# satoutahhaithem/gym

Measured on AMD Instinct MI355X. Metric: strategy-step param GB/s (%HBM/xGMI peak) + ms/outer step, GPT-2 124M, 1-8 GPUs, higher is better.
Workload: dtype f32

## Files before the change

### gym_amd/csrc/demo_wave.hip

```cpp
#include "ga_common.h"

namespace ga {
namespace dw {

constexpr int kWaves = 8;
constexpr int kThreads = 64 * kWaves;
constexpr int kLd = 65;
constexpr int kCand = 128;
static_assert(2 * (kCand + 64) >= 320, "the fallback top-k keeps its maps in lst[128..319]");

typedef float f32x16 __attribute__((ext_vector_type(16)));

#ifdef GA_DEMO_STAMPS
extern __device__ unsigned long long* g_demo_stamps_w;
#define DW_PH_DECL unsigned long long ph_acc[16] = {}, ph_last = __builtin_amdgcn_s_memtime()
#define DW_PH(i)                                                    \
    do {                                                            \
        const unsigned long long t_ = __builtin_amdgcn_s_memtime(); \
        ph_acc[i] += t_ - ph_last;                                  \
        ph_last = t_;                                               \
    } while (0)
#define DW_CNT(i) (ph_acc[i] += 1)
#define DW_PH_FLUSH()                                                                                       \
    do {                                                                                                    \
        if ((threadIdx.x & 63) == 0) {                                                                      \
            unsigned long long* row_ = g_demo_stamps_w + ((size_t)blockIdx.x * kWaves + (threadIdx.x >> 6)) * 16; \
            for (int i_ = 0; i_ < 16; ++i_) row_[i_] = ph_acc[i_];                                          \
        }                                                                                                   \
    } while (0)
#else
#define DW_PH_DECL do {} while (0)
#define DW_PH(i) do {} while (0)
#define DW_CNT(i) do {} while (0)
#define DW_PH_FLUSH() do {} while (0)
#endif

#define WAVE_LDS_SYNC() asm volatile("" ::: "memory")

__device__ __forceinline__ int lane_id() {
    int t = (int)threadIdx.x;
    asm volatile("" : "+v"(t));
    return t & 63;
}

__device__ __forceinline__ f32x16 zero16() {
    f32x16 a;
#pragma unroll
    for (int r = 0; r < 16; ++r) a[r] = 0.f;
    return a;
}

__device__ __forceinline__ f32x16 mfma(float a, float b, const f32x16& c) {
    return __builtin_amdgcn_mfma_f32_32x32x2f32(a, b, c, 0, 0, 0);
}

__device__ __forceinline__ constexpr int rowmap(int r, int h) { return (r & 3) + 8 * (r >> 2) + 4 * h; }

__device__ __forceinline__ int blk(int h, int q) { return h ? 4 + q : (q < 4 ? q : 8 + q); }

__device__ __forceinline__ int pi_col(int H, int m) { return 4 * blk((m >> 2) & 1, 4 * H + (m >> 3)) + (m & 3); }

__device__ __forceinline__ float basis64(const float* Hb, int i, int d) {
    const float v = Hb[(i < 32 ? i : 63 - i) * kLd + d];
    return (i >= 32 && (d & 1)) ? -v : v;
}

__device__ __forceinline__ uint32_t keyv(float v) { return (__float_as_uint(v) & 0x7fffffffu) + 1u; }

__device__ __forceinline__ int wave_excl_scan128(int v) {
    int r = 0;
#pragma unroll
    for (int b = 0; b < 7; ++b) {
        const uint64_t m = __ballot((v >> b) & 1);
        r += (int)__builtin_amdgcn_mbcnt_hi((uint32_t)(m >> 32), __builtin_amdgcn_mbcnt_lo((uint32_t)m, 0u)) << b;
    }
    return r;
}

__device__ __forceinline__ int wave_sum(int v) {
#pragma unroll
    for (int d = 32; d > 0; d >>= 1) v += __shfl_xor(v, d, 64);
    return v;
}

__device__ __forceinline__ int find_tensor(const ga_demo_tensor* __restrict__ T, int ntens, int tix, int chunk) {
    int lo = tix < 0 ? 0 : tix, hi = ntens - 1;
    while (lo < hi) {
        const int mid = (lo + hi + 1) >> 1;
        if (T[mid].chunk_start <= chunk) lo = mid;
        else hi = mid - 1;
    }
    return lo;
}

__device__ __forceinline__ void decode_wave_priority() {
    const int w = __builtin_amdgcn_readfirstlane((int)threadIdx.x >> 6);
    asm volatile("s_cmp_lt_u32 %0, 4\n\ts_cbranch_scc1 1f\n\ts_setprio 1\n1:" ::"s"(w) : "scc");
}

__device__ __forceinline__ uint32_t rdl(uint32_t v, int j) {
    return (uint32_t)__builtin_amdgcn_readlane((int)v, j);
}

struct ListLDS {
    uint32_t lst[2 * (kCand + 64)];
    uint32_t bm[128];
    uint32_t sm[4];
};

struct WaveLDS : ListLDS {
    float tile[64 * kLd];
};

__device__ __forceinline__ uint32_t lane_off(int s, int q, int l, int h, int stride) {
    return (uint32_t)((s ? 63 - l : l) * stride + 4 * blk(h, q));
}

template <typename T>
__device__ __forceinline__ const T* at_off(const T* pb, uint32_t off) {
    return reinterpret_cast<const T*>(reinterpret_cast<const char*>(pb) + (uint64_t)(uint32_t)(off * (uint32_t)sizeof(T)));
}
template <typename T>
__device__ __forceinline__ T* at_off(T* pb, uint32_t off) {
    return reinterpret_cast<T*>(reinterpret_cast<char*>(pb) + (uint64_t)(uint32_t)(off * (uint32_t)sizeof(T)));
}

template <typename T>
__device__ __forceinline__ void load_rows(const T* pb, int stride, int l, int h, bool vec, int nrows,
                                          float (&o)[2][8][4]) {
    if (vec && nrows == 64) {
#pragma unroll
        for (int s = 0; s < 2; ++s)
#pragma unroll
            for (int q = 0; q < 8; ++q)
                Vec4<T>::unpack(*reinterpret_cast<const typename Vec4<T>::type*>(at_off(pb, lane_off(s, q, l, h, stride))),
                                o[s][q]);
        return;
    }
#pragma unroll
    for (int s = 0; s < 2; ++s) {
        const bool live = (s ? 63 - l : l) < nrows;
#pragma unroll
        for (int q = 0; q < 8; ++q) {
            const T* a = at_off(pb, lane_off(s, q, l, h, stride));
            if (live && vec) {
                Vec4<T>::unpack(*reinterpret_cast<const typename Vec4<T>::type*>(a), o[s][q]);
            } else {
#pragma unroll
                for (int e = 0; e < 4; ++e) o[s][q][e] = live ? Elem<T>::load(a + e) : 0.f;
            }
        }
    }
}

template <typename T>
__device__ __forceinline__ void store_rows(T* pb, int stride, int l, int h, bool vec, int nrows,
                                           const float (&o)[2][8][4]) {
    if (vec && nrows == 64) {
#pragma unroll
        for (int s = 0; s < 2; ++s)
#pragma unroll
            for (int q = 0; q < 8; ++q)
                *reinterpret_cast<typename Vec4<T>::type*>(at_off(pb, lane_off(s, q, l, h, stride))) = Vec4<T>::pack(o[s][q]);
        return;
    }
#pragma unroll
    for (int s = 0; s < 2; ++s) {
        if ((s ? 63 - l : l) >= nrows) continue;
#pragma unroll
        for (int q = 0; q < 8; ++q) {
            T* a = at_off(pb, lane_off(s, q, l, h, stride));
            if (vec) {
                *reinterpret_cast<typename Vec4<T>::type*>(a) = Vec4<T>::pack(o[s][q]);
            } else {
#pragma unroll
                for (int e = 0; e < 4; ++e) Elem<T>::store(a + e, o[s][q][e]);
            }
        }
    }
}

template <typename T>
__device__ __forceinline__ void error_feedback(T* param, const T* grad, const T* delta, int stride, int l, int h,
                                               bool vec, int nrows, float lr, float decay, float wd_factor,
                                               float (&x)[2][8][4]) {
    if (wd_factor != 1.f) {
        load_rows(param, stride, l, h, vec, nrows, x);
#pragma unroll
        for (int s = 0; s < 2; ++s)
#pragma unroll
            for (int q = 0; q < 8; ++q)
#pragma unroll
                for (int e = 0; e < 4; ++e) x[s][q][e] *= wd_factor;
        store_rows(param, stride, l, h, vec, nrows, x);
    }
    float g[2][8][4];
    load_rows(delta, stride, l, h, vec, nrows, x);
    load_rows(grad, stride, l, h, vec, nrows, g);
#pragma unroll
    for (int s = 0; s < 2; ++s)
#pragma unroll
        for (int q = 0; q < 8; ++q)
#pragma unroll
            for (int e = 0; e < 4; ++e)
                x[s][q][e] = fmaf(lr, g[s][q][e], decay != 1.f ? x[s][q][e] * decay : x[s][q][e]);
}

__device__ __forceinline__ void row_product_half(const float (&xs)[8][4], const float* Hb, int l, int h,
                                                 f32x16 (&Ts)[2]) {
#pragma unroll
    for (int qc = 0; qc < 2; ++qc) {
        f32x16 acc = zero16();
#pragma unroll
        for (int t = 0; t < 16; ++t) {
            const int q = t >> 2, e = t & 3;
            const float u = xs[q][e], w = xs[7 - q][3 - e];
            const float a = qc ? u - w : u + w;
            acc = mfma(a, Hb[(16 * h + t) * kLd + 2 * l + qc], acc);
        }
        Ts[qc] = acc;
    }
}

__device__ __forceinline__ void row_product(const float (&x)[2][8][4], const float* Hb, int l, int h,
                                            f32x16 (&T)[2][2]) {
#pragma unroll
    for (int s = 0; s < 2; ++s) {
#pragma unroll
        for (int qc = 0; qc < 2; ++qc) {
            f32x16 acc = zero16();
#pragma unroll
            for (int t = 0; t < 16; ++t) {
                const int q = t >> 2, e = t & 3;
                const float u = x[s][q][e], w = x[s][7 - q][3 - e];
                const float a = qc ? u - w : u + w;
                acc = mfma(a, Hb[(16 * h + t) * kLd + 2 * l + qc], acc);
            }
            T[s][qc] = acc;
        }
    }
}

constexpr int kSynB = 4;

__device__ __forceinline__ void parity_lists(uint32_t epos, uint32_t ebits, bool ent, int lane, uint2* lstp,
                                             int& np0, int& np1) {
    const int pl = (int)((epos >> 6) & 1u);
    const uint64_t m0 = __ballot(ent && pl == 0), m1 = __ballot(ent && pl == 1);
    const uint64_t mm = pl ? m1 : m0;
    const int ix = (int)__builtin_amdgcn_mbcnt_hi((uint32_t)(mm >> 32), __builtin_amdgcn_mbcnt_lo((uint32_t)mm, 0u));
    const int E0 = __popcll(m0), E1 = __popcll(m1);
    const int P0 = (E0 + 1) & ~1, P1 = (E1 + 1) & ~1;
    WAVE_LDS_SYNC();
    if (ent) lstp[pl * 64 + ix] = make_uint2(epos, ebits);
    if (lane == 0 && E0 < P0) lstp[E0] = make_uint2(0u, 0u);
    if (lane == 1 && E1 < P1) lstp[64 + E1] = make_uint2(0u, 0u);
    WAVE_LDS_SYNC();
    np0 = P0 >> 1;
    np1 = P1 >> 1;
}

template <int B>
__device__ __forceinline__ void synth_batch(const uint2* lst, int q, int cH, int l, int h, const float* Hb,
                                            f32x16& acc) {
    uint2 e[B];
#pragma unroll
    for (int u = 0; u < B; ++u) e[u] = lst[2 * (q + u) + h];
    float a[B], b[B];
#pragma unroll
    for (int u = 0; u < B; ++u) {
        const int bq = (int)(e[u].x >> 6), dq = (int)(e[u].x & 63);
        a[u] = __uint_as_float(e[u].y) * basis64(Hb, cH, dq);
        b[u] = Hb[l * kLd + bq];
    }
#pragma unroll
    for (int u = 0; u < B; ++u) acc = mfma(a[u], b[u], acc);
}

__device__ __forceinline__ void synth_list(const uint2* lst, int np, int cH, int l, int h, const float* Hb,
                                           f32x16& acc) {
    static_assert(kSynB == 2 || kSynB == 4 || kSynB == 8, "synthesis tail handles 4/2/1 pairs");
    int q = 0;
    for (; q + kSynB <= np; q += kSynB) synth_batch<kSynB>(lst, q, cH, l, h, Hb, acc);
    const int rem = np - q;
    if (kSynB > 4 && (rem & 4)) {
        synth_batch<4>(lst, q, cH, l, h, Hb, acc);
        q += 4;
    }
    if (kSynB > 2 && (rem & 2)) {
        synth_batch<2>(lst, q, cH, l, h, Hb, acc);
        q += 2;
    }
    if (rem & 1) synth_batch<1>(lst, q, cH, l, h, Hb, acc);
}

__device__ __forceinline__ void synth_half(const uint2* lstp, int np0, int np1, int H, int l, int h,
                                           const float* Hb, f32x16& Re, f32x16& Ro) {
    const int cH = pi_col(H, l);
    Re = zero16();
    Ro = zero16();
    synth_list(lstp, np0, cH, l, h, Hb, Re);
    synth_list(lstp + 64, np1, cH, l, h, Hb, Ro);
}

__device__ __forceinline__ uint32_t coal_off(int i, int lane, int stride) {
    return (uint32_t)(((lane >> 4) + 4 * i) * stride + 4 * (lane & 15));
}

template <typename T, int I0 = 0, int NI = 16>
__device__ __forceinline__ void load_coal(const T* pb, int stride, bool vec, int lane, float (&o)[16][4]) {
    if (vec) {
#pragma unroll
        for (int i = I0; i < I0 + NI; ++i)
            Vec4<T>::unpack(*reinterpret_cast<const typename Vec4<T>::type*>(at_off(pb, coal_off(i, lane, stride))),
                            o[i]);
    } else {
#pragma unroll
        for (int i = I0; i < I0 + NI; ++i)
#pragma unroll
            for (int e = 0; e < 4; ++e) o[i][e] = Elem<T>::load(at_off(pb, coal_off(i, lane, stride)) + e);
    }
}

template <typename T>
__device__ __forceinline__ void store_vec(T* pb, uint32_t off, const typename Vec4<T>::type& v) {
    *reinterpret_cast<typename Vec4<T>::type*>(at_off(pb, off)) = v;
}

template <typename T>
__device__ __forceinline__ void store_coal(T* pb, int stride, bool vec, int lane, const float (&o)[16][4]) {
    if (vec) {
#pragma unroll
        for (int i = 0; i < 16; ++i) store_vec(pb, coal_off(i, lane, stride), Vec4<T>::pack(o[i]));
    } else {
#pragma unroll
        for (int i = 0; i < 16; ++i)
#pragma unroll
            for (int e = 0; e < 4; ++e) Elem<T>::store(at_off(pb, coal_off(i, lane, stride)) + e, o[i][e]);
    }
}

__device__ __forceinline__ int t4(int row, int cb) { return row * 16 + (cb ^ (row & 15)); }


template <typename T>
__device__ __forceinline__ void chunk64_tail(const f32x16 (&Y)[2][2], int k, T* delta, int cols, bool vec,
                                             int32_t* out_idx, float* out_val, const float* Hb, ListLDS& W,
                                             float4* tile
#ifdef GA_DEMO_STAMPS
                                             , unsigned long long (&ph_acc)[16], unsigned long long& ph_last
#endif
) {
    const int lane = lane_id(), l = lane & 31, h = lane >> 5;
    __builtin_amdgcn_s_setprio(1);
    auto posof = [&](int par, int qc, int r) -> uint32_t {
        return (uint32_t)((2 * rowmap(r, h) + par) * 64 + 2 * l + qc);
    };
    float mymaxf = 0.f;
#pragma unroll
    for (int par = 0; par < 2; ++par)
#pragma unroll
        for (int qc = 0; qc < 2; ++qc)
#pragma unroll
            for (int r = 0; r < 16; ++r) mymaxf = fmaxf(mymaxf, fabsf(Y[par][qc][r]));
    const uint32_t mymax = keyv(mymaxf);
    uint32_t T0 = 0;
#pragma unroll
    for (int bit = 30; bit >= 19; --bit) {
        const uint32_t cnd = T0 | (1u << bit);
        if (__popcll(__ballot(mymax >= cnd)) >= k) T0 = cnd;
    }
    if (T0 == 0u) T0 = 1u;
    const float T0f = __uint_as_float(T0 - 1u);
    int mine = 0;
#pragma unroll
    for (int par = 0; par < 2; ++par)
#pragma unroll
        for (int qc = 0; qc < 2; ++qc)
#pragma unroll
            for (int r = 0; r < 16; ++r) mine += fabsf(Y[par][qc][r]) >= T0f ? 1 : 0;
    const int excl = wave_excl_scan128(mine);
    const int incl = excl + mine;
    const int C = __builtin_amdgcn_readlane(incl, 63);
    DW_PH(10);
    W.bm[2 * lane] = 0u;
    W.bm[2 * lane + 1] = 0u;
    if (C <= kCand) {
        uint2* L2 = reinterpret_cast<uint2*>(W.lst);
        float T0c = T0f;
        asm volatile("" : "+v"(T0c));
        int at = excl;
#pragma unroll
        for (int par = 0; par < 2; ++par)
#pragma unroll
            for (int qc = 0; qc < 2; ++qc)
#pragma unroll
                for (int r = 0; r < 16; ++r) {
                    const float v = Y[par][qc][r];
                    const bool cnd = fabsf(v) >= T0c;
                    L2[cnd ? at : kCand + lane] = make_uint2(posof(par, qc, r), __float_as_uint(v));
                    at += cnd ? 1 : 0;
                }
        WAVE_LDS_SYNC();
        DW_PH(11);
        uint32_t pos[2], bits[2], key[2];
        bool ok[2];
#pragma unroll
        for (int e = 0; e < 2; ++e) {
            const int g = e * 64 + lane;
            ok[e] = g < C;
            const uint2 pb = L2[ok[e] ? g : kCand + lane];
            pos[e] = ok[e] ? pb.x : 0u;
            bits[e] = pb.y;
            key[e] = ok[e] ? keyv(__uint_as_float(pb.y)) : 0u;
            if (ok[e]) atomicOr(&W.bm[pos[e] >> 5], 1u << (pos[e] & 31));
        }
        WAVE_LDS_SYNC();
        const uint32_t w0 = W.bm[2 * lane], w1 = W.bm[2 * lane + 1];
        const int cnt = __popc(w0) + __popc(w1);
        const int pre = wave_excl_scan128(cnt);
        int rank[2];
#pragma unroll
        for (int e = 0; e < 2; ++e) {
            const int Lw = (int)(pos[e] >> 6);
            const uint64_t pair = ((uint64_t)(uint32_t)__shfl((int)w1, Lw, 64) << 32) |
                                  (uint32_t)__shfl((int)w0, Lw, 64);
            const int preL = __shfl(pre, Lw, 64);
            rank[e] = ok[e] ? preL + __popcll(pair & ((1ull << (pos[e] & 63)) - 1ull)) : 0x7fff;
        }
        DW_PH(12);
        uint32_t thr = 0;
        for (int bit = 31; bit >= 0; --bit) {
            const uint32_t cnd = thr | (1u << bit);
            if (__popcll(__ballot(key[0] >= cnd)) + __popcll(__ballot(key[1] >= cnd)) >= k) thr = cnd;
        }
        const int need = k - __popcll(__ballot(key[0] > thr)) - __popcll(__ballot(key[1] > thr));
        const uint64_t q0 = __ballot(key[0] == thr), q1 = __ballot(key[1] == thr);
        bool sel[2];
        if (__popcll(q0) + __popcll(q1) == need) {
            sel[0] = key[0] >= thr;
            sel[1] = key[1] >= thr;
        } else {
            int tr[2] = {0, 0};
            for (uint64_t m = q0; m; m &= m - 1) {
                const int rj = __builtin_amdgcn_readlane(rank[0], __builtin_ctzll(m));
                tr[0] += rj < rank[0];
                tr[1] += rj < rank[1];
            }
            for (uint64_t m = q1; m; m &= m - 1) {
                const int rj = __builtin_amdgcn_readlane(rank[1], __builtin_ctzll(m));
                tr[0] += rj < rank[0];
                tr[1] += rj < rank[1];
            }
            sel[0] = key[0] > thr || (key[0] == thr && tr[0] < need);
            sel[1] = key[1] > thr || (key[1] == thr && tr[1] < need);
        }
        DW_PH(13);
        if (lane < 4) W.sm[lane] = 0u;
        WAVE_LDS_SYNC();
#pragma unroll
        for (int e = 0; e < 2; ++e)
            if (sel[e]) atomicOr(&W.sm[rank[e] >> 5], 1u << (rank[e] & 31));
        WAVE_LDS_SYNC();
        const uint64_t m0 = ((uint64_t)W.sm[1] << 32) | W.sm[0], m1 = ((uint64_t)W.sm[3] << 32) | W.sm[2];
#pragma unroll
        for (int e = 0; e < 2; ++e) {
            if (sel[e]) {
                const int r = rank[e];
                const int slot = r < 64 ? __popcll(m0 & ((1ull << r) - 1ull))
                                        : __popcll(m0) + __popcll(m1 & ((1ull << (r - 64)) - 1ull));
                W.lst[2 * slot] = pos[e];
                W.lst[2 * slot + 1] = bits[e];
                out_idx[slot] = (int32_t)pos[e];
                out_val[slot] = __uint_as_float(bits[e]);
            }
        }
        WAVE_LDS_SYNC();
    } else {
        DW_CNT(8);
        auto opq = [](float v) {
            asm volatile("" : "+v"(v));
            return v;
        };
        auto lane_pos = [&]() {
            uint32_t lp = (uint32_t)(512 * h + 2 * l);
            asm volatile("" : "+v"(lp));
            return lp;
        };
        auto pos_c = [](int par, int qc, int r) -> uint32_t {
            return (uint32_t)((2 * ((r & 3) + 8 * (r >> 2)) + par) * 64 + qc);
        };
        uint32_t thr = 0;
        for (int bit = 31; bit >= 0; --bit) {
            const uint32_t cnd = thr | (1u << bit);
            const float f = __uint_as_float(cnd - 1u);
            int cl = 0;
#pragma unroll
            for (int par = 0; par < 2; ++par)
#pragma unroll
                for (int qc = 0; qc < 2; ++qc)
#pragma unroll
                    for (int r = 0; r < 16; ++r) cl += fabsf(opq(Y[par][qc][r])) >= f ? 1 : 0;
            if (wave_sum(cl) >= k) thr = cnd;
        }
        int gl = 0;
        {
            const uint32_t lp = lane_pos();
#pragma unroll
            for (int par = 0; par < 2; ++par)
#pragma unroll
                for (int qc = 0; qc < 2; ++qc)
#pragma unroll
                    for (int r = 0; r < 16; ++r) {
                        const uint32_t kv = keyv(opq(Y[par][qc][r]));
                        gl += kv > thr ? 1 : 0;
                        if (kv == thr) {
                            const uint32_t p = lp + pos_c(par, qc, r);
                            atomicOr(&W.bm[p >> 5], 1u << (p & 31));
                        }
                    }
        }
        const int need = k - wave_sum(gl);
        WAVE_LDS_SYNC();
        uint32_t* preL = W.lst + 128;
        {
            const uint32_t w0 = W.bm[2 * lane], w1 = W.bm[2 * lane + 1];
            preL[lane] = (uint32_t)wave_excl_scan128(__popc(w0) + __popc(w1));
        }
        WAVE_LDS_SYNC();
        uint32_t* sel = W.lst + 192;
        sel[2 * lane] = 0u;
        sel[2 * lane + 1] = 0u;
        WAVE_LDS_SYNC();
        {
            const uint32_t lp = lane_pos();
#pragma unroll
            for (int par = 0; par < 2; ++par)
#pragma unroll
                for (int qc = 0; qc < 2; ++qc)
#pragma unroll
                    for (int r = 0; r < 16; ++r) {
                        const uint32_t kv = keyv(opq(Y[par][qc][r]));
                        const uint32_t p = lp + pos_c(par, qc, r);
                        bool s = kv > thr;
                        if (kv == thr) {
                            const uint32_t Lw = p >> 6;
                            const uint64_t pair = ((uint64_t)W.bm[2 * Lw + 1] << 32) | W.bm[2 * Lw];
                            const int tr = (int)preL[Lw] + __popcll(pair & ((1ull << (p & 63)) - 1ull));
                            s = tr < need;
                        }
                        if (s) atomicOr(&sel[p >> 5], 1u << (p & 31));
                    }
        }
        WAVE_LDS_SYNC();
        {
            const uint32_t w0 = sel[2 * lane], w1 = sel[2 * lane + 1];
            preL[lane] = (uint32_t)wave_excl_scan128(__popc(w0) + __popc(w1));
        }
        WAVE_LDS_SYNC();
        {
            const uint32_t lp = lane_pos();
#pragma unroll
            for (int par = 0; par < 2; ++par)
#pragma unroll
                for (int qc = 0; qc < 2; ++qc)
#pragma unroll
                    for (int r = 0; r < 16; ++r) {
                        const uint32_t p = lp + pos_c(par, qc, r);
                        const uint32_t Lw = p >> 6;
                        const uint64_t pair = ((uint64_t)sel[2 * Lw + 1] << 32) | sel[2 * Lw];
                        if ((pair >> (p & 63)) & 1ull) {
                            const int slot = (int)preL[Lw] + __popcll(pair & ((1ull << (p & 63)) - 1ull));
                            const float v = opq(Y[par][qc][r]);
                            W.lst[2 * slot] = p;
                            W.lst[2 * slot + 1] = __float_as_uint(v);
                            out_idx[slot] = (int32_t)p;
                            out_val[slot] = v;
                        }
                    }
        }
        WAVE_LDS_SYNC();
    }
    DW_PH(3);
    __builtin_amdgcn_s_setprio(0);
    uint2* lstp = reinterpret_cast<uint2*>(W.lst);
    int np0, np1;
    parity_lists(lane < k ? W.lst[2 * lane] : 0u, lane < k ? W.lst[2 * lane + 1] : 0u, lane < k, lane, lstp, np0,
                 np1);
#pragma unroll
    for (int H = 0; H < 2; ++H) {
        f32x16 Re, Ro;
        synth_half(lstp, np0, np1, H, l, h, Hb, Re, Ro);
#pragma unroll
        for (int qq = 0; qq < 4; ++qq)
#pragma unroll
            for (int s = 0; s < 2; ++s) {
                float4& v = tile[t4(s ? 63 - l : l, blk(h, 4 * H + qq))];
                float4 o = v;
                const int r = 4 * qq;
                o.x -= s ? Re[r] - Ro[r] : Re[r] + Ro[r];
                o.y -= s ? Re[r + 1] - Ro[r + 1] : Re[r + 1] + Ro[r + 1];
                o.z -= s ? Re[r + 2] - Ro[r + 2] : Re[r + 2] + Ro[r + 2];
                o.w -= s ? Re[r + 3] - Ro[r + 3] : Re[r + 3] + Ro[r + 3];
                v = o;
            }
        DW_PH(4);
    }
    WAVE_LDS_SYNC();
    {
        float o[16][4];
#pragma unroll
        for (int i = 0; i < 16; ++i) {
            const float4 v = tile[t4((lane >> 4) + 4 * i, lane & 15)];
            o[i][0] = v.x;
            o[i][1] = v.y;
            o[i][2] = v.z;
            o[i][3] = v.w;
        }
        store_coal(delta, cols, vec, lane, o);
    }
    WAVE_LDS_SYNC();
    DW_PH(5);
}

template <typename T>
__device__ __forceinline__ void chunk64(const ga_demo_tensor& td, int c, T* param, const T* grad, T* delta,
                                        int32_t* out_idx, float* out_val, float lr, float decay, float wd_factor,
                                        int ptr_vec, const float* Hb, WaveLDS& W
#ifdef GA_DEMO_STAMPS
                                        , unsigned long long (&ph_acc)[16], unsigned long long& ph_last
#endif
) {
    const int cy = c / td.gx, cx = c - cy * td.gx;
    const int64_t base = td.offset + (int64_t)cy * 64 * td.cols + (int64_t)cx * 64;
    param += base;
    grad += base;
    delta += base;
    const bool vec = ptr_vec && (td.offset % 4 == 0) && (td.cols % 4 == 0);
    float4* tile = reinterpret_cast<float4*>(W.tile);
    {
        const int lane = lane_id();
        if (wd_factor != 1.f) {
            float pv[16][4];
            load_coal(param, td.cols, vec, lane, pv);
#pragma unroll
            for (int i = 0; i < 16; ++i)
#pragma unroll
                for (int e = 0; e < 4; ++e) pv[i][e] *= wd_factor;
            store_coal(param, td.cols, vec, lane, pv);
        }
    }
    f32x16 Y[2][2];
    {
        const int lane = lane_id(), l = lane & 31, h = lane >> 5;
        float Dv[16][4], Gv[16][4];
        __builtin_amdgcn_s_setprio(2);
        load_coal<T, 0, 8>(delta, td.cols, vec, lane, Dv);
        load_coal<T, 0, 8>(grad, td.cols, vec, lane, Gv);
        __builtin_amdgcn_sched_barrier(0);
        load_coal<T, 8, 8>(delta, td.cols, vec, lane, Dv);
        load_coal<T, 8, 8>(grad, td.cols, vec, lane, Gv);
#pragma unroll
        for (int i = 0; i < 8; ++i)
            asm volatile("" : "+v"(Dv[i][0]), "+v"(Dv[i][1]), "+v"(Dv[i][2]), "+v"(Dv[i][3]), "+v"(Gv[i][0]),
                              "+v"(Gv[i][1]), "+v"(Gv[i][2]), "+v"(Gv[i][3])::"memory");
        __builtin_amdgcn_s_setprio(0);
        f32x16 Tm[2][2];
#pragma unroll
        for (int s = 0; s < 2; ++s) {
#pragma unroll
            for (int i = 8 * s; i < 8 * s + 8; ++i) {
                if (s == 1)
                    asm volatile("" : "+v"(Dv[i][0]), "+v"(Dv[i][1]), "+v"(Dv[i][2]), "+v"(Dv[i][3]),
                                      "+v"(Gv[i][0]), "+v"(Gv[i][1]), "+v"(Gv[i][2]), "+v"(Gv[i][3]));
                float v[4];
#pragma unroll
                for (int e = 0; e < 4; ++e) v[e] = fmaf(lr, Gv[i][e], Dv[i][e] * decay);
                tile[t4((lane >> 4) + 4 * i, lane & 15)] = make_float4(v[0], v[1], v[2], v[3]);
            }
            WAVE_LDS_SYNC();
            float xs[8][4];
#pragma unroll
            for (int q = 0; q < 8; ++q) {
                const float4 v = tile[t4(s ? 63 - l : l, blk(h, q))];
                xs[q][0] = v.x;
                xs[q][1] = v.y;
                xs[q][2] = v.z;
                xs[q][3] = v.w;
            }
            row_product_half(xs, Hb, l, h, Tm[s]);
            if (s == 0) __builtin_amdgcn_sched_barrier(0);
        }
        DW_PH(1);
#pragma unroll
        for (int qc = 0; qc < 2; ++qc) {
#pragma unroll
            for (int par = 0; par < 2; ++par) {
                f32x16 acc = zero16();
#pragma unroll
                for (int t = 0; t < 16; ++t) {
                    const float u = Tm[0][qc][t], w = Tm[1][qc][t];
                    acc = mfma(Hb[rowmap(t, h) * kLd + 2 * l + par], par ? u - w : u + w, acc);
                }
                Y[par][qc] = acc;
            }
        }
    }
    DW_PH(2);
    chunk64_tail<T>(Y, td.k, delta, td.cols, vec, out_idx, out_val, Hb, W, tile
#ifdef GA_DEMO_STAMPS
                    , ph_acc, ph_last
#endif
    );
}

template <typename T>
__device__ __forceinline__ void rowgroup(const ga_demo_rowgroup& rg, T* param, const T* grad, T* delta,
                                         int32_t* pay_idx, float* pay_val, float lr, float decay,
                                         float wd_factor, int ptr_vec, const float* Hb, WaveLDS& W
#ifdef GA_DEMO_STAMPS
                                         , unsigned long long (&ph_acc)[16], unsigned long long& ph_last
#endif
) {
    const int rows = rg.rows, k = rg.k;
    const bool vec = ptr_vec && (rg.offset % 4 == 0);
    param += rg.offset;
    grad += rg.offset;
    delta += rg.offset;
    float x[2][8][4];
    {
        const int lane = lane_id(), l = lane & 31, h = lane >> 5;
        error_feedback(param, grad, delta, 64, l, h, vec, rows, lr, decay, wd_factor, x);
    }
    DW_PH(6);
    {
        const int lane = lane_id(), l = lane & 31, h = lane >> 5;
        f32x16 Tm[2][2];
        row_product(x, Hb, l, h, Tm);
#pragma unroll
        for (int s = 0; s < 2; ++s)
#pragma unroll
            for (int qc = 0; qc < 2; ++qc)
#pragma unroll
                for (int r = 0; r < 16; ++r) {
                    const int i = rowmap(r, h);
                    W.tile[(s ? 63 - i : i) * kLd + 2 * l + qc] = Tm[s][qc][r];
                }
    }
    WAVE_LDS_SYNC();
    {
        const int L = lane_id();
        float* trow = W.tile + L * kLd;
        float yr[64];
#pragma unroll
        for (int t = 0; t < 64; ++t) yr[t] = trow[t];
        uint32_t thr = 0;
        for (int bit = 31; bit >= 0; --bit) {
            const uint32_t cnd = thr | (1u << bit);
            int cl = 0;
#pragma unroll
            for (int t = 0; t < 64; ++t) cl += fabsf(yr[t]) >= __uint_as_float(cnd - 1u) ? 1 : 0;
            if (cl >= k) thr = cnd;
        }
        int gl = 0;
#pragma unroll
        for (int t = 0; t < 64; ++t) gl += keyv(yr[t]) > thr ? 1 : 0;
        int need = k - gl;
        int slot = 0;
        const bool live = L < rows;
        int32_t* oi = pay_idx + (int64_t)L * k;
        float* ov = pay_val + (int64_t)L * k;
#pragma unroll
        for (int t = 0; t < 64; ++t) {
            const uint32_t kv = keyv(yr[t]);
            const bool tie = kv == thr && need > 0;
            const bool s = kv > thr || tie;
            need -= tie ? 1 : 0;
            if (s && live) {
                oi[slot] = t;
                ov[slot] = yr[t];
            }
            slot += s ? 1 : 0;
            trow[t] = s ? yr[t] : 0.f;
        }
    }
    WAVE_LDS_SYNC();
    {
        const int lane = lane_id(), l = lane & 31, h = lane >> 5;
        const int c0 = pi_col(0, l), c1 = pi_col(1, l);
#pragma unroll
        for (int s = 0; s < 2; ++s) {
            const float* yrow = W.tile + (s ? 63 - l : l) * kLd;
            f32x16 r0 = zero16(), r1 = zero16();
#pragma unroll
            for (int t = 0; t < 32; ++t) {
                const int d = 2 * t + h;
                const float yv = yrow[d];
                r0 = mfma(basis64(Hb, c0, d), yv, r0);
                r1 = mfma(basis64(Hb, c1, d), yv, r1);
            }
#pragma unroll
            for (int q = 0; q < 8; ++q)
#pragma unroll
                for (int e = 0; e < 4; ++e) x[s][q][e] -= (q < 4 ? r0 : r1)[4 * (q & 3) + e];
        }
        store_rows(delta, 64, l, h, vec, rows, x);
    }
    WAVE_LDS_SYNC();
    DW_PH(7);
}

template <typename T>
__global__ __launch_bounds__(kThreads) void encode_kernel(
    const ga_demo_tensor* __restrict__ tens, int ntens, int nchunks, const ga_demo_rowgroup* __restrict__ groups,
    int ngroups, const float* __restrict__ F64, T* param0, const T* __restrict__ grad0, T* delta0, int64_t ld,
    int64_t K, float lr, float decay, float wd_factor, int32_t* payload0, int64_t pstride, int64_t M, int ptr_vec) {
    __shared__ float Hb[32 * kLd];
    __shared__ WaveLDS wl[kWaves];
    __shared__ int next_job;
    for (int q = threadIdx.x; q < 32 * 64; q += kThreads) Hb[(q >> 6) * kLd + (q & 63)] = F64[q];
    next_job = 0;
    __syncthreads();
    const int wid = __builtin_amdgcn_readfirstlane((int)threadIdx.x >> 6);
    WaveLDS& W = wl[wid];
    DW_PH_DECL;
    const int64_t n64 = (int64_t)nchunks * K;
    const int64_t stride = (int64_t)gridDim.x * kWaves;
    const int64_t b8 = (int64_t)blockIdx.x * kWaves;
    const int64_t g_total = (int64_t)ngroups * K;
    const uint32_t st = (uint32_t)stride;
    uint32_t nc32 = 0;
#pragma unroll
    for (int w = 0; w < kWaves; ++w)
        if (b8 + w < n64) nc32 += ((uint32_t)(n64 - (b8 + w)) + st - 1u) / st;
    const int64_t nc = nc32;
    const int64_t ng = (int64_t)blockIdx.x < g_total
                           ? ((uint32_t)(g_total - blockIdx.x) + gridDim.x - 1u) / gridDim.x : 0;
    const int64_t nt = nc + ng;
    int tix = -1;
    int64_t last_rep = -1;
    while (true) {
        int tv = 0;
        if (lane_id() == 0) tv = atomicAdd(&next_job, 1);
        const int64_t t = __builtin_amdgcn_readfirstlane(tv);
        if (t >= nt) break;
        const int64_t job = t < ng ? n64 + (int64_t)blockIdx.x + t * gridDim.x
                                   : b8 + ((t - ng) & 7) + ((t - ng) >> 3) * stride;
        if (job < n64) {
            const int64_t rep = job / nchunks;
            const int chunk = (int)(job - rep * nchunks);
            if (rep != last_rep) {
                tix = -1;
                last_rep = rep;
            }
            tix = find_tensor(tens, ntens, tix, chunk);
            const ga_demo_tensor td = tens[tix];
            const int c = chunk - td.chunk_start;
            int32_t* pi = payload0 + rep * pstride + td.payload_off + (int64_t)c * td.k;
            float* pv = reinterpret_cast<float*>(payload0 + rep * pstride + M) + td.payload_off + (int64_t)c * td.k;
            chunk64<T>(td, c, param0 + rep * ld, grad0 + rep * ld, delta0 + rep * ld, pi, pv, lr, decay, wd_factor,
                       ptr_vec, Hb, W
#ifdef GA_DEMO_STAMPS
                       , ph_acc, ph_last
#endif
            );
            DW_CNT(9);
        } else {
            const int64_t j = job - n64;
            const int64_t rep = j / ngroups;
            const int g = (int)(j - rep * ngroups);
            const ga_demo_rowgroup rg = groups[g];
            rowgroup<T>(rg, param0 + rep * ld, grad0 + rep * ld, delta0 + rep * ld,
                        payload0 + rep * pstride + rg.payload_off,
                        reinterpret_cast<float*>(payload0 + rep * pstride + M) + rg.payload_off, lr, decay,
                        wd_factor, ptr_vec, Hb, W
#ifdef GA_DEMO_STAMPS
                        , ph_acc, ph_last
#endif
            );
        }
    }
    DW_PH_FLUSH();
}

template <typename T>
static int launch(const ga_demo_tensor* tens, int32_t ntens, int32_t nchunks, const ga_demo_rowgroup* groups,
                  int32_t ngroups, const float* F64, void* param, const void* grad, void* delta, int64_t K,
                  int64_t ld, float lr, float decay, float wd_factor, int32_t* payload, int64_t pstride, int64_t M,
                  int ptr_vec, hipStream_t stream) {
    static const int cus = [] {
        int dev = 0, n = 0;
        (void)hipGetDevice(&dev);
        (void)hipDeviceGetAttribute(&n, hipDeviceAttributeMultiprocessorCount, dev);
        return n > 0 ? n : 256;
    }();
    auto kern = encode_kernel<T>;
    static const int resident = [&] {
        int per_cu = 0;
        (void)hipOccupancyMaxActiveBlocksPerMultiprocessor(&per_cu, kern, kThreads, 0);
        return (per_cu > 0 ? per_cu : 1) * cus;
    }();
    const int64_t jobs = ((int64_t)nchunks + ngroups) * K;
    const int64_t want = (jobs + kWaves - 1) / kWaves;
    const int grid = (int)(want < resident ? want : resident);
    if (grid <= 0) return GA_OK;
    hipLaunchKernelGGL(kern, dim3(grid), dim3(kThreads), 0, stream, tens, ntens, nchunks, groups, ngroups, F64,
                       (T*)param, (const T*)grad, (T*)delta, ld, K, lr, decay, wd_factor, payload, pstride, M,
                       ptr_vec);
    return GA_OK;
}

constexpr int kMaxSrc = 15;

struct DecLDS {
    float tile[64 * 64];
    uint32_t aux[512];
};

__device__ __forceinline__ int fidx(int row, int col) { return row * 64 + 4 * ((col >> 2) ^ (row & 15)) + (col & 3); }

__device__ __forceinline__ float sgnf(float g) {
    return fabsf(g) > 0.f ? __builtin_copysignf(1.f, g) : 0.f;
}

template <typename T>
using PRaw = typename Vec4<T>::type[16];

template <typename T>
__device__ __forceinline__ void load_coal_raw(const T* pb, int stride, bool vec, int lane, PRaw<T>& o) {
    if (vec) {
#pragma unroll
        for (int i = 0; i < 16; ++i)
            o[i] = *reinterpret_cast<const typename Vec4<T>::type*>(at_off(pb, coal_off(i, lane, stride)));
    } else {
#pragma unroll
        for (int i = 0; i < 16; ++i) {
            float f[4];
#pragma unroll
            for (int e = 0; e < 4; ++e) f[e] = Elem<T>::load(at_off(pb, coal_off(i, lane, stride)) + e);
            o[i] = Vec4<T>::pack(f);
        }
    }
}

template <typename T, bool NTS = false>
__device__ __forceinline__ void store_quad(T* pb, int i, int stride, bool vec, int lane, const float (&f)[4]) {
    T* a = at_off(pb, coal_off(i, lane, stride));
    if (vec) {
        if constexpr (NTS) stream_store(reinterpret_cast<typename Vec4<T>::type*>(a), Vec4<T>::pack(f));
        else store_vec(pb, coal_off(i, lane, stride), Vec4<T>::pack(f));
    } else {
#pragma unroll
        for (int e = 0; e < 4; ++e) Elem<T>::store(a + e, f[e]);
    }
}

template <typename T, bool NTS = false>
__device__ __forceinline__ void sign_update(const float4* tile, T* pr, T* gr, int stride, bool vec, float lr,
                                            int lane, PRaw<T>& raw) {
    if constexpr (sizeof(typename Vec4<T>::type) < 16) {
#pragma unroll
        for (int i = 0; i < 16; ++i) {
            const float4 v = tile[t4((lane >> 4) + 4 * i, lane & 15)];
            float f[4];
            Vec4<T>::unpack(raw[i], f);
            f[0] = fmaf(-lr, v.x, f[0]);
            f[1] = fmaf(-lr, v.y, f[1]);
            f[2] = fmaf(-lr, v.z, f[2]);
            f[3] = fmaf(-lr, v.w, f[3]);
            store_quad(pr, i, stride, vec, lane, f);
        }
        if (gr) {
#pragma unroll
            for (int i = 0; i < 16; ++i) {
                const float4 v = tile[t4((lane >> 4) + 4 * i, lane & 15)];
                const float f[4] = {v.x, v.y, v.z, v.w};
                store_quad<T, NTS>(gr, i, stride, vec, lane, f);
            }
        }
    } else {
#pragma unroll
        for (int i = 0; i < 16; ++i) {
            const float4 v = tile[t4((lane >> 4) + 4 * i, lane & 15)];
            raw[i].x = fmaf(-lr, v.x, raw[i].x);
            raw[i].y = fmaf(-lr, v.y, raw[i].y);
            raw[i].z = fmaf(-lr, v.z, raw[i].z);
            raw[i].w = fmaf(-lr, v.w, raw[i].w);
        }
        if (vec) {
#pragma unroll
            for (int i = 0; i < 16; ++i) *reinterpret_cast<float4*>(at_off(pr, coal_off(i, lane, stride))) = raw[i];
        } else {
#pragma unroll
            for (int i = 0; i < 16; ++i) {
                const float f[4] = {raw[i].x, raw[i].y, raw[i].z, raw[i].w};
                store_quad(pr, i, stride, vec, lane, f);
            }
        }
        if (gr) {
#pragma unroll
            for (int i = 0; i < 16; ++i) {
                const float4 v = tile[t4((lane >> 4) + 4 * i, lane & 15)];
                const float f[4] = {v.x, v.y, v.z, v.w};
                store_quad<T, NTS>(gr, i, stride, vec, lane, f);
            }
        }
    }
}

template <typename T, bool NTS = false>
__device__ __forceinline__ void apply_signs(const float4* tile, T* param, T* grad, int64_t K, int64_t ld, int stride,
                                            bool vec, int nrows, float lr, int lane, PRaw<T>& pre, bool lean = false) {
    if (nrows == 64) {
        sign_update<T, NTS>(tile, param, grad, stride, vec, lr, lane, pre);
        if (lean) {
            for (int64_t r = 1; r < K; ++r) {
#pragma unroll 4
                for (int i = 0; i < 16; ++i) {
                    const float4 v = tile[t4((lane >> 4) + 4 * i, lane & 15)];
                    T* a = at_off(param + r * ld, coal_off(i, lane, stride));
                    float f[4];
                    if (vec) {
                        Vec4<T>::unpack(*reinterpret_cast<const typename Vec4<T>::type*>(a), f);
                    } else {
#pragma unroll
                        for (int e = 0; e < 4; ++e) f[e] = Elem<T>::load(a + e);
                    }
                    f[0] = fmaf(-lr, v.x, f[0]);
                    f[1] = fmaf(-lr, v.y, f[1]);
                    f[2] = fmaf(-lr, v.z, f[2]);
                    f[3] = fmaf(-lr, v.w, f[3]);
                    store_quad(param + r * ld, i, stride, vec, lane, f);
                    if (grad) {
                        const float g4[4] = {v.x, v.y, v.z, v.w};
                        store_quad(grad + r * ld, i, stride, vec, lane, g4);
                    }
                }
            }
            return;
        }
        for (int64_t r = 1; r < K; ++r) {
            PRaw<T> p;
            load_coal_raw(param + r * ld, stride, vec, lane, p);
            sign_update<T, NTS>(tile, param + r * ld, grad ? grad + r * ld : nullptr, stride, vec, lr, lane, p);
        }
        return;
    }
    for (int64_t r = 0; r < K; ++r) {
#pragma unroll
        for (int i0 = 0; i0 < 16; i0 += 8) {
            float f[8][4];
#pragma unroll
            for (int i = 0; i < 8; ++i) {
                const bool live = (lane >> 4) + 4 * (i0 + i) < nrows;
                const T* a = at_off(param + r * ld, coal_off(i0 + i, lane, stride));
#pragma unroll
                for (int e = 0; e < 4; ++e) f[i][e] = live ? Elem<T>::load(a + e) : 0.f;
            }
#pragma unroll
            for (int ii = 0; ii < 8; ++ii) {
                const int i = i0 + ii;
                if ((lane >> 4) + 4 * i >= nrows) continue;
                const float4 v = tile[t4((lane >> 4) + 4 * i, lane & 15)];
                const float sg[4] = {v.x, v.y, v.z, v.w};
                T* a = at_off(param + r * ld, coal_off(i, lane, stride));
#pragma unroll
                for (int e = 0; e < 4; ++e) Elem<T>::store(a + e, fmaf(-lr, sg[e], f[ii][e]));
                if (grad) {
                    T* gq = at_off(grad + r * ld, coal_off(i, lane, stride));
#pragma unroll
                    for (int e = 0; e < 4; ++e) Elem<T>::store(gq + e, sg[e]);
                }
            }
        }
    }
}

constexpr int kGrpBatch = 16;

template <typename RowOf>
__device__ __forceinline__ void scatter_sources(DecLDS& W, const int32_t* __restrict__ payload, int64_t pstride,
                                                int64_t M, int64_t e0, int S, int n, int nvalid, RowOf row_of,
                                                int lane) {
    for (int s = 0; s < S; ++s) {
        const int32_t* pi = payload + (int64_t)s * pstride + e0;
        const float* pv = reinterpret_cast<const float*>(payload + (int64_t)s * pstride + M) + e0;
        for (int j0 = 0; j0 < n; j0 += 64 * kGrpBatch) {
            int xb[kGrpBatch];
            float vb[kGrpBatch];
#pragma unroll
            for (int u = 0; u < kGrpBatch; ++u) {
                const int j = j0 + 64 * u + lane;
                xb[u] = j < n ? pi[j] : -1;
                vb[u] = j < n ? pv[j] : 0.f;
            }
#pragma unroll
            for (int u = 0; u < kGrpBatch; ++u) {
                const int x = xb[u];
                if ((unsigned)x < (unsigned)nvalid) {
                    const int j = j0 + 64 * u + lane;
                    const int row = row_of(j, x), col = nvalid == 64 ? x : (x & 63);
                    atomicAdd(&W.tile[fidx(row, col)], vb[u]);
                    const int cid = row * 64 + col;
                    atomicAdd(&W.aux[cid >> 3], 1u << (4 * (cid & 7)));
                }
            }
        }
        WAVE_LDS_SYNC();
    }
}

__device__ __forceinline__ float mean_of(float sum, uint32_t cw) {
    const uint32_t n = cw & 15u;
    return n > 1u ? sum / (float)n : sum;
}

template <int MS>
struct DecIn {
    int xs[MS];
    float vs[MS];
};

__device__ __forceinline__ int64_t chunk_base(const ga_demo_tensor& td, int c) {
// ... 358 lines not shown
```

Baseline: 2502.

## Split DCT basis into parity planes in LDS and streamline top-k candidate selection

Stores the shared basis matrix as two parity planes (even/odd columns, row stride 33) instead of interleaved rows of stride 65. The goal is to avoid LDS bank conflicts when lanes read columns 2*l+qc, and the synthesis list entries now carry precomputed plane offsets. Candidate compaction now walks a per-lane bitmask with clz and a select tree instead of writing all 64 values with dummy stores. Top-k selection is templated for one or two candidate rows, breaks ties by position instead of a precomputed rank, and drops the second selection bitmap pass.

```diff
diff --git a/gym_amd/csrc/demo_wave.hip b/gym_amd/csrc/demo_wave.hip
--- a/gym_amd/csrc/demo_wave.hip
+++ b/gym_amd/csrc/demo_wave.hip
@@ -60,8 +60,31 @@
 
 __device__ __forceinline__ int pi_col(int H, int m) { return 4 * blk((m >> 2) & 1, 4 * H + (m >> 3)) + (m & 3); }
 
+struct BasisRows {
+    static constexpr int kFloats = 32 * kLd;
+    __device__ static __forceinline__ int at(int i, int d) { return i * kLd + d; }
+    __device__ static __forceinline__ int at2(int i, int j, int par) { return i * kLd + 2 * j + par; }
+    __device__ static __forceinline__ uint32_t entry(uint32_t p) { return p; }
+    __device__ static __forceinline__ int ent_b(uint32_t x) { return (int)(x >> 6); }
+    __device__ static __forceinline__ int ent_d(uint32_t x) { return (int)(x & 63); }
+    __device__ static __forceinline__ bool ent_d_odd(uint32_t x) { return x & 1u; }
+};
+struct BasisPlanes {
+    static constexpr int kRow = 33, kPlane = 32 * kRow, kFloats = 2 * kPlane;
+    __device__ static __forceinline__ int at(int i, int d) { return (d & 1) * kPlane + i * kRow + (d >> 1); }
+    __device__ static __forceinline__ int at2(int i, int j, int par) { return par * kPlane + i * kRow + j; }
+    __device__ static __forceinline__ uint32_t entry(uint32_t p) {
+        return (uint32_t)at(0, (int)(p >> 6)) << 16 | (uint32_t)at(0, (int)(p & 63));
+    }
+    __device__ static __forceinline__ int ent_b(uint32_t x) { return (int)(x >> 16); }
+    __device__ static __forceinline__ int ent_d(uint32_t x) { return (int)(x & 0xffffu); }
+    __device__ static __forceinline__ bool ent_d_odd(uint32_t x) { return (x & 0xffffu) >= (uint32_t)kPlane; }
+};
+using EncBasis = BasisPlanes;
+
+template <class BL = BasisRows>
 __device__ __forceinline__ float basis64(const float* Hb, int i, int d) {
-    const float v = Hb[(i < 32 ? i : 63 - i) * kLd + d];
+    const float v = Hb[BL::at(i < 32 ? i : 63 - i, d)];
     return (i >= 32 && (d & 1)) ? -v : v;
 }
 
@@ -102,10 +125,22 @@
     return (uint32_t)__builtin_amdgcn_readlane((int)v, j);
 }
 
+__device__ __forceinline__ float sel16(const f32x16& a, bool b0, bool b1, bool b2, bool b3) {
+    const float p0 = b0 ? a[1] : a[0], p1 = b0 ? a[3] : a[2], p2 = b0 ? a[5] : a[4], p3 = b0 ? a[7] : a[6];
+    const float p4 = b0 ? a[9] : a[8], p5 = b0 ? a[11] : a[10], p6 = b0 ? a[13] : a[12], p7 = b0 ? a[15] : a[14];
+    const float q0 = b1 ? p1 : p0, q1 = b1 ? p3 : p2, q2 = b1 ? p5 : p4, q3 = b1 ? p7 : p6;
+    const float s0 = b2 ? q1 : q0, s1 = b2 ? q3 : q2;
+    return b3 ? s1 : s0;
+}
+
+template <int N>
+struct IntC {
+    static constexpr int value = N;
+};
+
 struct ListLDS {
     uint32_t lst[2 * (kCand + 64)];
     uint32_t bm[128];
-    uint32_t sm[4];
 };
 
 struct WaveLDS : ListLDS {
@@ -206,6 +241,7 @@
                 x[s][q][e] = fmaf(lr, g[s][q][e], decay != 1.f ? x[s][q][e] * decay : x[s][q][e]);
 }
 
+template <class BL>
 __device__ __forceinline__ void row_product_half(const float (&xs)[8][4], const float* Hb, int l, int h,
                                                  f32x16 (&Ts)[2]) {
 #pragma unroll
@@ -216,12 +252,13 @@
             const int q = t >> 2, e = t & 3;
             const float u = xs[q][e], w = xs[7 - q][3 - e];
             const float a = qc ? u - w : u + w;
-            acc = mfma(a, Hb[(16 * h + t) * kLd + 2 * l + qc], acc);
+            acc = mfma(a, Hb[BL::at2(16 * h + t, l, qc)], acc);
         }
         Ts[qc] = acc;
     }
 }
 
+template <class BL>
 __device__ __forceinline__ void row_product(const float (&x)[2][8][4], const float* Hb, int l, int h,
                                             f32x16 (&T)[2][2]) {
 #pragma unroll
@@ -234,7 +271,7 @@
                 const int q = t >> 2, e = t & 3;
                 const float u = x[s][q][e], w = x[s][7 - q][3 - e];
                 const float a = qc ? u - w : u + w;
-                acc = mfma(a, Hb[(16 * h + t) * kLd + 2 * l + qc], acc);
+                acc = mfma(a, Hb[BL::at2(16 * h + t, l, qc)], acc);
             }
             T[s][qc] = acc;
         }
@@ -243,6 +280,7 @@
 
 constexpr int kSynB = 4;
 
+template <class BL = BasisRows>
 __device__ __forceinline__ void parity_lists(uint32_t epos, uint32_t ebits, bool ent, int lane, uint2* lstp,
                                              int& np0, int& np1) {
     const int pl = (int)((epos >> 6) & 1u);
@@ -252,7 +290,7 @@
     const int E0 = __popcll(m0), E1 = __popcll(m1);
     const int P0 = (E0 + 1) & ~1, P1 = (E1 + 1) & ~1;
     WAVE_LDS_SYNC();
-    if (ent) lstp[pl * 64 + ix] = make_uint2(epos, ebits);
+    if (ent) lstp[pl * 64 + ix] = make_uint2(BL::entry(epos), ebits);
     if (lane == 0 && E0 < P0) lstp[E0] = make_uint2(0u, 0u);
     if (lane == 1 && E1 < P1) lstp[64 + E1] = make_uint2(0u, 0u);
     WAVE_LDS_SYNC();
@@ -260,7 +298,7 @@
     np1 = P1 >> 1;
 }
 
-template <int B>
+template <int B, class BL>
 __device__ __forceinline__ void synth_batch(const uint2* lst, int q, int cH, int l, int h, const float* Hb,
                                             f32x16& acc) {
     uint2 e[B];
@@ -269,38 +307,40 @@
     float a[B], b[B];
 #pragma unroll
     for (int u = 0; u < B; ++u) {
-        const int bq = (int)(e[u].x >> 6), dq = (int)(e[u].x & 63);
-        a[u] = __uint_as_float(e[u].y) * basis64(Hb, cH, dq);
-        b[u] = Hb[l * kLd + bq];
+        const float f = Hb[BL::at(cH < 32 ? cH : 63 - cH, 0) + BL::ent_d(e[u].x)];
+        a[u] = __uint_as_float(e[u].y) * ((cH >= 32 && BL::ent_d_odd(e[u].x)) ? -f : f);
+        b[u] = Hb[BL::at(l, 0) + BL::ent_b(e[u].x)];
     }
 #pragma unroll
     for (int u = 0; u < B; ++u) acc = mfma(a[u], b[u], acc);
 }
 
+template <class BL>
 __device__ __forceinline__ void synth_list(const uint2* lst, int np, int cH, int l, int h, const float* Hb,
                                            f32x16& acc) {
     static_assert(kSynB == 2 || kSynB == 4 || kSynB == 8, "synthesis tail handles 4/2/1 pairs");
     int q = 0;
-    for (; q + kSynB <= np; q += kSynB) synth_batch<kSynB>(lst, q, cH, l, h, Hb, acc);
+    for (; q + kSynB <= np; q += kSynB) synth_batch<kSynB, BL>(lst, q, cH, l, h, Hb, acc);
     const int rem = np - q;
     if (kSynB > 4 && (rem & 4)) {
-        synth_batch<4>(lst, q, cH, l, h, Hb, acc);
+        synth_batch<4, BL>(lst, q, cH, l, h, Hb, acc);
         q += 4;
     }
     if (kSynB > 2 && (rem & 2)) {
-        synth_batch<2>(lst, q, cH, l, h, Hb, acc);
+        synth_batch<2, BL>(lst, q, cH, l, h, Hb, acc);
         q += 2;
     }
-    if (rem & 1) synth_batch<1>(lst, q, cH, l, h, Hb, acc);
-}
-
+    if (rem & 1) synth_batch<1, BL>(lst, q, cH, l, h, Hb, acc);
+}
+
+template <class BL = BasisRows>
 __device__ __forceinline__ void synth_half(const uint2* lstp, int np0, int np1, int H, int l, int h,
                                            const float* Hb, f32x16& Re, f32x16& Ro) {
     const int cH = pi_col(H, l);
     Re = zero16();
     Ro = zero16();
-    synth_list(lstp, np0, cH, l, h, Hb, Re);
-    synth_list(lstp + 64, np1, cH, l, h, Hb, Ro);
+    synth_list<BL>(lstp, np0, cH, l, h, Hb, Re);
+    synth_list<BL>(lstp + 64, np1, cH, l, h, Hb, Ro);
 }
 
 __device__ __forceinline__ uint32_t coal_off(int i, int lane, int stride) {
@@ -353,9 +393,6 @@
 ) {
     const int lane = lane_id(), l = lane & 31, h = lane >> 5;
     __builtin_amdgcn_s_setprio(1);
-    auto posof = [&](int par, int qc, int r) -> uint32_t {
-        return (uint32_t)((2 * rowmap(r, h) + par) * 64 + 2 * l + qc);
-    };
     float mymaxf = 0.f;
 #pragma unroll
     for (int par = 0; par < 2; ++par)
@@ -372,13 +409,14 @@
     }
     if (T0 == 0u) T0 = 1u;
     const float T0f = __uint_as_float(T0 - 1u);
-    int mine = 0;
+    uint32_t cm[2] = {0u, 0u};
 #pragma unroll
     for (int par = 0; par < 2; ++par)
 #pragma unroll
         for (int qc = 0; qc < 2; ++qc)
 #pragma unroll
-            for (int r = 0; r < 16; ++r) mine += fabsf(Y[par][qc][r]) >= T0f ? 1 : 0;
+            for (int r = 0; r < 16; ++r) cm[par] = cm[par] + cm[par] + (fabsf(Y[par][qc][r]) >= T0f ? 1u : 0u);
+    const int mine = __popc(cm[0]) + __popc(cm[1]);
     const int excl = wave_excl_scan128(mine);
     const int incl = excl + mine;
     const int C = __builtin_amdgcn_readlane(incl, 63);
@@ -387,95 +425,102 @@
     W.bm[2 * lane + 1] = 0u;
     if (C <= kCand) {
         uint2* L2 = reinterpret_cast<uint2*>(W.lst);
-        float T0c = T0f;
-        asm volatile("" : "+v"(T0c));
-        int at = excl;
-#pragma unroll
-        for (int par = 0; par < 2; ++par)
-#pragma unroll
-            for (int qc = 0; qc < 2; ++qc)
-#pragma unroll
-                for (int r = 0; r < 16; ++r) {
-                    const float v = Y[par][qc][r];
-                    const bool cnd = fabsf(v) >= T0c;
-                    L2[cnd ? at : kCand + lane] = make_uint2(posof(par, qc, r), __float_as_uint(v));
-                    at += cnd ? 1 : 0;
-                }
+        {
+            int at = excl;
+            while (__ballot((cm[0] | cm[1]) != 0u)) {
+                const bool has = (cm[0] | cm[1]) != 0u, first = cm[0] != 0u;
+                const uint32_t w = first ? cm[0] : cm[1];
+                const uint32_t tp = (uint32_t)__clz((int)w) & 31u;
+                const uint32_t left = w & ~(0x80000000u >> tp);
+                cm[0] = first ? left : cm[0];
+                cm[1] = first ? cm[1] : left;
+                const bool b0 = tp & 1u, b1 = tp & 2u, b2 = tp & 4u, b3 = tp & 8u, b4 = tp & 16u;
+                const float v0 = b4 ? sel16(Y[0][1], b0, b1, b2, b3) : sel16(Y[0][0], b0, b1, b2, b3);
+                const float v1 = b4 ? sel16(Y[1][1], b0, b1, b2, b3) : sel16(Y[1][0], b0, b1, b2, b3);
+                const uint32_t r = tp & 15u, qc = tp >> 4, par = first ? 0u : 1u;
+                const uint32_t pos = (2u * ((r & 3u) + 8u * (r >> 2) + 4u * (uint32_t)h) + par) * 64u +
+                                     2u * (uint32_t)l + qc;
+                if (has) L2[at] = make_uint2(pos, __float_as_uint(first ? v0 : v1));
+                at += 1;
+            }
+        }
         WAVE_LDS_SYNC();
         DW_PH(11);
-        uint32_t pos[2], bits[2], key[2];
-        bool ok[2];
-#pragma unroll
-        for (int e = 0; e < 2; ++e) {
-            const int g = e * 64 + lane;
-            ok[e] = g < C;
-            const uint2 pb = L2[ok[e] ? g : kCand + lane];
-            pos[e] = ok[e] ? pb.x : 0u;
-            bits[e] = pb.y;
-            key[e] = ok[e] ? keyv(__uint_as_float(pb.y)) : 0u;
-            if (ok[e]) atomicOr(&W.bm[pos[e] >> 5], 1u << (pos[e] & 31));
-        }
-        WAVE_LDS_SYNC();
-        const uint32_t w0 = W.bm[2 * lane], w1 = W.bm[2 * lane + 1];
-        const int cnt = __popc(w0) + __popc(w1);
-        const int pre = wave_excl_scan128(cnt);
-        int rank[2];
-#pragma unroll
-        for (int e = 0; e < 2; ++e) {
-            const int Lw = (int)(pos[e] >> 6);
-            const uint64_t pair = ((uint64_t)(uint32_t)__shfl((int)w1, Lw, 64) << 32) |
-                                  (uint32_t)__shfl((int)w0, Lw, 64);
-            const int preL = __shfl(pre, Lw, 64);
-            rank[e] = ok[e] ? preL + __popcll(pair & ((1ull << (pos[e] & 63)) - 1ull)) : 0x7fff;
-        }
-        DW_PH(12);
-        uint32_t thr = 0;
-        for (int bit = 31; bit >= 0; --bit) {
-            const uint32_t cnd = thr | (1u << bit);
-            if (__popcll(__ballot(key[0] >= cnd)) + __popcll(__ballot(key[1] >= cnd)) >= k) thr = cnd;
-        }
-        const int need = k - __popcll(__ballot(key[0] > thr)) - __popcll(__ballot(key[1] > thr));
-        const uint64_t q0 = __ballot(key[0] == thr), q1 = __ballot(key[1] == thr);
-        bool sel[2];
-        if (__popcll(q0) + __popcll(q1) == need) {
-            sel[0] = key[0] >= thr;
-            sel[1] = key[1] >= thr;
-        } else {
-            int tr[2] = {0, 0};
-            for (uint64_t m = q0; m; m &= m - 1) {
-                const int rj = __builtin_amdgcn_readlane(rank[0], __builtin_ctzll(m));
-                tr[0] += rj < rank[0];
-                tr[1] += rj < rank[1];
-            }
-            for (uint64_t m = q1; m; m &= m - 1) {
-                const int rj = __builtin_amdgcn_readlane(rank[1], __builtin_ctzll(m));
-                tr[0] += rj < rank[0];
-                tr[1] += rj < rank[1];
-            }
-            sel[0] = key[0] > thr || (key[0] == thr && tr[0] < need);
-            sel[1] = key[1] > thr || (key[1] == thr && tr[1] < need);
-        }
-        DW_PH(13);
-        if (lane < 4) W.sm[lane] = 0u;
-        WAVE_LDS_SYNC();
-#pragma unroll
-        for (int e = 0; e < 2; ++e)
-            if (sel[e]) atomicOr(&W.sm[rank[e] >> 5], 1u << (rank[e] & 31));
-        WAVE_LDS_SYNC();
-        const uint64_t m0 = ((uint64_t)W.sm[1] << 32) | W.sm[0], m1 = ((uint64_t)W.sm[3] << 32) | W.sm[2];
-#pragma unroll
-        for (int e = 0; e < 2; ++e) {
-            if (sel[e]) {
-                const int r = rank[e];
-                const int slot = r < 64 ? __popcll(m0 & ((1ull << r) - 1ull))
-                                        : __popcll(m0) + __popcll(m1 & ((1ull << (r - 64)) - 1ull));
-                W.lst[2 * slot] = pos[e];
-                W.lst[2 * slot + 1] = bits[e];
-                out_idx[slot] = (int32_t)pos[e];
-                out_val[slot] = __uint_as_float(bits[e]);
-            }
-        }
-        WAVE_LDS_SYNC();
+        auto select = [&](auto ec) {
+            constexpr int E = decltype(ec)::value;
+            uint32_t pos[E], bits[E], key[E];
+            bool ok[E];
+#pragma unroll
+            for (int e = 0; e < E; ++e) {
+                const int g = e * 64 + lane;
+                ok[e] = g < C;
+                const uint2 pb = L2[ok[e] ? g : kCand + lane];
+                pos[e] = ok[e] ? pb.x : 0u;
+                bits[e] = pb.y;
+                key[e] = ok[e] ? keyv(__uint_as_float(pb.y)) : 0u;
+            }
+            DW_PH(12);
+            auto count = [&](auto pred) {
+                int n = 0;
+#pragma unroll
+                for (int e = 0; e < E; ++e) n += __popcll(__ballot(pred(key[e])));
+                return n;
+            };
+            uint32_t thr = 0;
+            for (int bit = 31; bit >= 0; --bit) {
+                const uint32_t cnd = thr | (1u << bit);
+                if (count([&](uint32_t kv) { return kv >= cnd; }) >= k) thr = cnd;
+            }
+            const int need = k - count([&](uint32_t kv) { return kv > thr; });
+            uint64_t q[E];
+            int nq = 0;
+#pragma unroll
+            for (int e = 0; e < E; ++e) {
+                q[e] = __ballot(key[e] == thr);
+                nq += __popcll(q[e]);
+            }
+            bool sel[E];
+            if (nq == need) {
+#pragma unroll
+                for (int e = 0; e < E; ++e) sel[e] = key[e] >= thr;
+            } else {
+                int tr[E];
+#pragma unroll
+                for (int e = 0; e < E; ++e) tr[e] = 0;
+#pragma unroll
+                for (int e2 = 0; e2 < E; ++e2)
+                    for (uint64_t m = q[e2]; m; m &= m - 1) {
+                        const uint32_t pj = rdl(pos[e2], __builtin_ctzll(m));
+#pragma unroll
+                        for (int e = 0; e < E; ++e) tr[e] += pj < pos[e];
+                    }
+#pragma unroll
+                for (int e = 0; e < E; ++e) sel[e] = key[e] > thr || (key[e] == thr && tr[e] < need);
+            }
+            DW_PH(13);
+#pragma unroll
+            for (int e = 0; e < E; ++e)
+                if (sel[e]) atomicOr(&W.bm[pos[e] >> 5], 1u << (pos[e] & 31));
+            WAVE_LDS_SYNC();
+            const uint32_t w0 = W.bm[2 * lane], w1 = W.bm[2 * lane + 1];
+            const int pre = wave_excl_scan128(__popc(w0) + __popc(w1));
+#pragma unroll
+            for (int e = 0; e < E; ++e) {
+                const int Lw = (int)(pos[e] >> 6);
+                const uint64_t pair = ((uint64_t)(uint32_t)__shfl((int)w1, Lw, 64) << 32) |
+                                      (uint32_t)__shfl((int)w0, Lw, 64);
+                const int slot = __shfl(pre, Lw, 64) + __popcll(pair & ((1ull << (pos[e] & 63)) - 1ull));
+                if (sel[e]) {
+                    W.lst[2 * slot] = pos[e];
+                    W.lst[2 * slot + 1] = bits[e];
+                    out_idx[slot] = (int32_t)pos[e];
+                    out_val[slot] = __uint_as_float(bits[e]);
+                }
+            }
+            WAVE_LDS_SYNC();
+        };
+        if (C <= 64) select(IntC<1>{});
+        else select(IntC<2>{});
     } else {
         DW_CNT(8);
         auto opq = [](float v) {
@@ -585,12 +630,12 @@
     __builtin_amdgcn_s_setprio(0);
     uint2* lstp = reinterpret_cast<uint2*>(W.lst);
     int np0, np1;
-    parity_lists(lane < k ? W.lst[2 * lane] : 0u, lane < k ? W.lst[2 * lane + 1] : 0u, lane < k, lane, lstp, np0,
-                 np1);
+    parity_lists<EncBasis>(lane < k ? W.lst[2 * lane] : 0u, lane < k ? W.lst[2 * lane + 1] : 0u, lane < k, lane,
+                           lstp, np0, np1);
 #pragma unroll
     for (int H = 0; H < 2; ++H) {
         f32x16 Re, Ro;
-        synth_half(lstp, np0, np1, H, l, h, Hb, Re, Ro);
+        synth_half<EncBasis>(lstp, np0, np1, H, l, h, Hb, Re, Ro);
 #pragma unroll
         for (int qq = 0; qq < 4; ++qq)
 #pragma unroll
@@ -688,7 +733,7 @@
                 xs[q][2] = v.z;
                 xs[q][3] = v.w;
             }
-            row_product_half(xs, Hb, l, h, Tm[s]);
+            row_product_half<EncBasis>(xs, Hb, l, h, Tm[s]);
             if (s == 0) __builtin_amdgcn_sched_barrier(0);
         }
         DW_PH(1);
@@ -700,7 +745,7 @@
 #pragma unroll
                 for (int t = 0; t < 16; ++t) {
                     const float u = Tm[0][qc][t], w = Tm[1][qc][t];
-                    acc = mfma(Hb[rowmap(t, h) * kLd + 2 * l + par], par ? u - w : u + w, acc);
+                    acc = mfma(Hb[EncBasis::at2(rowmap(t, h), l, par)], par ? u - w : u + w, acc);
                 }
                 Y[par][qc] = acc;
             }
@@ -736,7 +781,7 @@
     {
         const int lane = lane_id(), l = lane & 31, h = lane >> 5;
         f32x16 Tm[2][2];
-        row_product(x, Hb, l, h, Tm);
+        row_product<EncBasis>(x, Hb, l, h, Tm);
 #pragma unroll
         for (int s = 0; s < 2; ++s)
 #pragma unroll
@@ -796,8 +841,8 @@
             for (int t = 0; t < 32; ++t) {
                 const int d = 2 * t + h;
                 const float yv = yrow[d];
-                r0 = mfma(basis64(Hb, c0, d), yv, r0);
-                r1 = mfma(basis64(Hb, c1, d), yv, r1);
+                r0 = mfma(basis64<EncBasis>(Hb, c0, d), yv, r0);
+                r1 = mfma(basis64<EncBasis>(Hb, c1, d), yv, r1);
             }
 #pragma unroll
             for (int q = 0; q < 8; ++q)
@@ -815,10 +860,10 @@
     const ga_demo_tensor* __restrict__ tens, int ntens, int nchunks, const ga_demo_rowgroup* __restrict__ groups,
     int ngroups, const float* __restrict__ F64, T* param0, const T* __restrict__ grad0, T* delta0, int64_t ld,
     int64_t K, float lr, float decay, float wd_factor, int32_t* payload0, int64_t pstride, int64_t M, int ptr_vec) {
-    __shared__ float Hb[32 * kLd];
+    __shared__ float Hb[EncBasis::kFloats];
     __shared__ WaveLDS wl[kWaves];
     __shared__ int next_job;
-    for (int q = threadIdx.x; q < 32 * 64; q += kThreads) Hb[(q >> 6) * kLd + (q & 63)] = F64[q];
+    for (int q = threadIdx.x; q < 32 * 64; q += kThreads) Hb[EncBasis::at(q >> 6, q & 63)] = F64[q];
     next_job = 0;
     __syncthreads();
     const int wid = __builtin_amdgcn_readfirstlane((int)threadIdx.x >> 6);
```

New measurement: 2499. About the same (-0.1%).
